# pasqal-io/Pulser

Hardware: NVIDIA H100
Metric: time-steps/s (1 ns sampling intervals of the Sequence evolved per second) (higher is better)
Workload: dtype f64 (complex128)

## Files before the change

### include/pulser_b200.h

```cpp
#ifndef PULSER_B200_H
#define PULSER_B200_H

#include <stdint.h>

#ifdef __cplusplus
extern "C" {
#endif

#define PB200_OK 0
#define PB200_ERR_INVALID -1
#define PB200_ERR_CUDA -2
#define PB200_ERR_UNSUPPORTED -3
#define PB200_ERR_STATE -4

#define PB200_MAX_QUDITS 40
#define PB200_MAX_DRIVES 3

typedef struct pb200_plan pb200_plan;

typedef struct pb200_drive_desc {
    int32_t state_to;
    int32_t state_from;
    int32_t uniform;
    int32_t reserved;
// ... 122 lines not shown
int pb200_shards_energy(pb200_plan** plans, int32_t count, double t_us,
                        double* energy, double* h2);
int pb200_shards_expect(pb200_plan** plans, int32_t count,
                        const pb200_op_terms* op, double* out);

int pb200_host_interpolate(const double* x, const double* y, int32_t n,
                           int32_t order, const double* tq, int32_t nq,
                           double* out);
int pb200_host_moments(const double* x, const double* y, int32_t n,
                       int32_t order, double a, double b, double* out4);
int pb200_host_taylor_fit(const double* x, const double* y, int32_t n,
                          int32_t order, double a, double h, int32_t p,
                          double* coeffs, double* resid);
int pb200_host_taylor_separable(const double* coef, const double* det,
                                int32_t n_traj, int32_t n_qudits,
                                int32_t n_times, int32_t* separable,
                                double* a_out, double* c_out, double* m_out);
int pb200_host_taylor_shapes(const double* coef, const double* det,
                             int32_t n_traj, int32_t n_qudits, int32_t n_times,
                             int32_t max_shapes, int32_t* n_shapes,
                             double* a_out, double* c_out, double* m_out);
int pb200_host_taylor_order(double h, const double* m, int32_t p, double tol,
                            int32_t* order_out, double* tail_out);
int pb200_host_chebyshev(double rho, double tol, double* out, int32_t cap,
                         int32_t* count);

#ifdef __cplusplus
}
#endif
#endif
```

### pulser_b200/_lib.py

```python
from __future__ import annotations

import ctypes as C
import os

_HERE = os.path.dirname(os.path.abspath(__file__))
LIB_PATH = os.path.join(_HERE, "libpulser_b200.so")

PB200_MAX_DRIVES = 3


class DriveDesc(C.Structure):
    _fields_ = [
        ("state_to", C.c_int32),
        ("state_from", C.c_int32),
        ("uniform", C.c_int32),
        ("reserved", C.c_int32),
    ]


class PlanDesc(C.Structure):
    _fields_ = [
        ("n_qudits", C.c_int32),
        ("dim", C.c_int32),
        ("n_times", C.c_int32),
# ... 100 lines not shown
        "pb200_bench_apply": (
            C.c_int, [vp, C.c_double, C.c_int32, dp, C.POINTER(C.c_int64)]),
        "pb200_plan_create_shard": (C.c_int, [C.POINTER(vp), C.POINTER(PlanDesc), C.c_int32, C.c_int32]),
        "pb200_shards_link": (C.c_int, [C.POINTER(vp), C.c_int32]),
        "pb200_shards_propagate": (
            C.c_int, [C.POINTER(vp), C.c_int32, C.c_double, C.c_double, C.POINTER(RunOpts), C.POINTER(RunStats)]),
        "pb200_shards_apply_h": (C.c_int, [C.POINTER(vp), C.c_int32, C.c_double, dp, dp]),
        "pb200_shards_energy": (C.c_int, [C.POINTER(vp), C.c_int32, C.c_double, dp, dp]),
        "pb200_shards_expect": (C.c_int, [C.POINTER(vp), C.c_int32, C.POINTER(OpTermsDesc), dp]),
        "pb200_host_interpolate": (
            C.c_int, [dp, dp, C.c_int32, C.c_int32, dp, C.c_int32, dp]),
        "pb200_host_moments": (
            C.c_int, [dp, dp, C.c_int32, C.c_int32, C.c_double, C.c_double, dp]),
        "pb200_host_chebyshev": (
            C.c_int, [C.c_double, C.c_double, dp, C.c_int32, C.POINTER(C.c_int32)]),
        "pb200_host_taylor_fit": (
            C.c_int, [dp, dp, C.c_int32, C.c_int32, C.c_double, C.c_double, C.c_int32, dp, dp]),
        "pb200_host_taylor_separable": (
            C.c_int, [dp, dp, C.c_int32, C.c_int32, C.c_int32, C.POINTER(C.c_int32), dp, dp, dp]),
        "pb200_host_taylor_shapes": (
            C.c_int, [dp, dp, C.c_int32, C.c_int32, C.c_int32, C.c_int32, C.POINTER(C.c_int32), dp, dp, dp]),
        "pb200_host_taylor_order": (
            C.c_int, [C.c_double, dp, C.c_int32, C.c_double, C.POINTER(C.c_int32), dp]),
    }
    for name, (res, args) in sig.items():
        fn = getattr(lib, name)
        fn.restype = res
        fn.argtypes = args
    return lib


EXPORTED_SYMBOLS = [
    "pb200_version", "pb200_last_error", "pb200_device_count",
    "pb200_plan_create", "pb200_plan_destroy", "pb200_plan_set_stream",
    "pb200_plan_set_interaction", "pb200_plan_set_xy", "pb200_plan_set_slm_mask", "pb200_plan_set_drive", "pb200_plan_set_dissipator", "pb200_plan_set_collapse",
    "pb200_plan_jump_counts", "pb200_state_set",
    "pb200_state_get", "pb200_state_probabilities", "pb200_state_norm2",
    "pb200_state_occupation", "pb200_state_correlation", "pb200_state_energy", "pb200_state_overlap", "pb200_state_expect", "pb200_state_sample", "pb200_state_copy", "pb200_state_device_ptr", "pb200_propagate", "pb200_apply_h",
    "pb200_coefficients_at", "pb200_bench_apply", "pb200_host_interpolate",
    "pb200_host_moments", "pb200_host_chebyshev", "pb200_host_taylor_fit", "pb200_host_taylor_order", "pb200_host_taylor_separable",
    "pb200_host_taylor_shapes",
    "pb200_plan_create_shard", "pb200_shards_link", "pb200_shards_propagate", "pb200_shards_apply_h", "pb200_shards_energy",
    "pb200_shards_expect",
]

lib = _load()


class PB200Error(RuntimeError):
    def __init__(self, code: int, msg: str):
        super().__init__(f"pulser_b200 error {code}: {msg}")
        self.code = code


def check(code: int) -> None:
    if code != 0:
        raise PB200Error(code, lib.pb200_last_error().decode("utf-8", "replace"))
```

### pulser_b200/csrc/kernels.cuh

```cuda
#pragma once
#include <cuda_runtime.h>
#include <stdint.h>
#include <type_traits>

namespace pb200 {

struct c2 { double x, y; };

__host__ __device__ inline c2 cmul(c2 a, c2 b) { return {a.x * b.x - a.y * b.y, a.x * b.y + a.y * b.x}; }
__host__ __device__ inline c2 cadd(c2 a, c2 b) { return {a.x + b.x, a.y + b.y}; }

struct PassGeom {
    int n_bits;
    int lo_bits;
    int hi_shift;
    int hi_bits;
    uint32_t tile_flip_mask;
    unsigned long long extra_mask;
    int first_pass;
};

struct StageCoef {
    c2 c_psi, c_b2, c_g;
};
// ... 1418 lines not shown
    for (long long idx = blockIdx.x * (long long)blockDim.x + threadIdx.x; idx < D;
         idx += (long long)gridDim.x * blockDim.x) {
        int cnt = 0;
        long long rem = off + idx;
        for (int k = 0; k < n; ++k) { cnt += ((int)(rem % dim) == rstate); rem /= dim; }
        const double v = dint[idx];
        unsigned long long* pmin = reinterpret_cast<unsigned long long*>(mins + cnt);
        unsigned long long old = *pmin;
        while (__longlong_as_double((long long)old) > v) {
            unsigned long long assumed = old;
            old = atomicCAS(pmin, assumed, (unsigned long long)__double_as_longlong(v));
            if (old == assumed) break;
        }
        unsigned long long* pmax = reinterpret_cast<unsigned long long*>(maxs + cnt);
        old = *pmax;
        while (__longlong_as_double((long long)old) < v) {
            unsigned long long assumed = old;
            old = atomicCAS(pmax, assumed, (unsigned long long)__double_as_longlong(v));
            if (old == assumed) break;
        }
    }
}

__global__ void bitstring_weights_kernel(const c2* psi, double* weights, long long D, int n, int dim, int one_digit,
                                         long long off) {
    for (long long s = blockIdx.x * (long long)blockDim.x + threadIdx.x; s < D;
         s += (long long)gridDim.x * blockDim.x) {
        const c2 v = psi[s];
        const double p = v.x * v.x + v.y * v.y;
        long long rem = off + s, b = 0;
        for (int k = n - 1; k >= 0; --k) {
            if ((int)(rem % dim) == one_digit) b |= 1LL << (n - 1 - k);
            rem /= dim;
        }
        if (dim == 2) weights[b & (D - 1)] = p;
        else atomicAdd(weights + b, p);
    }
}

__global__ void occupation_kernel(const c2* psi, double* occ, long long D, int n, int dim, int digit, long long off) {
    extern __shared__ double socc[];
    for (int i = threadIdx.x; i < n; i += blockDim.x) socc[i] = 0.0;
    __syncthreads();
    const long long traj = blockIdx.y;
    for (long long s = blockIdx.x * (long long)blockDim.x + threadIdx.x; s < D;
         s += (long long)gridDim.x * blockDim.x) {
// ... 451 lines not shown
```

### pulser_b200/csrc/plan.cu

```cuda
#include <cuda_runtime.h>

#include <algorithm>
#include <deque>
#include <map>
#include <memory>
#include <mutex>
#include <unordered_map>
#include <cmath>
#include <complex>
#include <cstdarg>
#include <cstdio>
#include <cstdlib>
#include <cstring>
#include <stdexcept>
#include <string>
#include <vector>

#include "../../include/pulser_b200.h"
#include "kernels.cuh"
#include "spline.hpp"
#include <cub/device/device_scan.cuh>
#include <nvtx3/nvToolsExt.h>
#include <random>

namespace pb200 {

// ... 230 lines not shown
    std::vector<double> times;
    int n = 0, dim = 0, B = 1;
    long long D = 0;
    int n_drives = 0;
    cudaStream_t stream = nullptr;
    struct OwnedStream {
        cudaStream_t s = nullptr;
        OwnedStream() = default;
        OwnedStream(const OwnedStream&) = delete;
        OwnedStream& operator=(const OwnedStream&) = delete;
        ~OwnedStream() { reset(); }
        void reset() {
            if (s) { cudaStreamSynchronize(s); cudaStreamDestroy(s); s = nullptr; }
        }
    } owned_stream;
    DevBuf<c2> buf[3];
    DevBuf<c2> aux[6];
    int cur = 0;
    DevBuf<double> dint;
    bool dint_shared = true;
    bool has_interaction = false;
    DevBuf<double> d_table;
    DevBuf<double> d_scratch;
    std::vector<std::vector<DriveTables>> tabs;
    std::vector<std::vector<bool>> tabs_set;
    std::vector<double> dmin_cnt, dmax_cnt;
    std::vector<double> dmin_traj, dmax_traj;
    bool state_set = false;
    int sm_count = 132;
    std::vector<std::vector<cplx>> diss_gen;
    DevBuf<c2> kry; int kry_cap = 0;
    DevBuf<double> d_kry;
    int m_last = 8;
    bool use_krylov = false;
    long long kry_iters = 0;
    bool has_diss = false;
    struct DissTaylor {
        bool ok = false;
        const char* why = "";
        c2 dw[4] = {}, df[4] = {};
        bool flip = false;
        double norm = 0.0;
    } diss_tay;
    std::vector<std::vector<cplx>> jump_ops;
    std::vector<std::vector<double>> jump_ldl;
    std::vector<std::vector<cplx>> jump_ldl_full;
// ... 1825 lines not shown
    return out;
}

static int taylor_order(double h, const std::vector<double>& mj, double tol, double& tail_out) {
    const int p = (int)mj.size() - 1;
    std::vector<double> y(1, 1.0);
    const int kcap = 1200;
    for (int k = 0; k < kcap; ++k) {
        double s = 0.0;
        for (int j = 0; j <= std::min(p, k); ++j) s += mj[j] * y[k - j];
        y.push_back(h * s / (k + 1));
        if (k > 8 && y.back() < 1e-40 && y.back() < y[k]) break;
    }
    double tail = 0.0;
    int kk = (int)y.size() - 1;
    for (; kk >= 1; --kk) {
        if (tail + y[kk] > tol) break;
        tail += y[kk];
    }
    tail_out = tail;
    return std::max(kk, 1);
}

static void launch_taylor_order(const Plan& P, bool tiled, const TaylorArgs& a, bool cplx) {
    const bool diss = a.n_pair > 0;
    if (!tiled) {
        const dim3 grid((unsigned)((P.D + 255) / 256), (unsigned)P.B);
        if (diss && !cplx) stage_d2_taylor_small_kernel<false, true><<<grid, 256, 0, P.stream>>>(a);
        else if (diss) fail(PB200_ERR_UNSUPPORTED, "no Taylor stage kernel for a dissipator with a complex drive");
        else if (cplx) stage_d2_taylor_small_kernel<true><<<grid, 256, 0, P.stream>>>(a);
        else stage_d2_taylor_small_kernel<false><<<grid, 256, 0, P.stream>>>(a);
        return;
    }
    const bool uniform = !a.table || (a.tab_shapes && P.tay.drive_uniform);
    const bool real_g = uniform && !cplx && a.unit.y == 0.0;
    const bool shard = a.shard_bits > 0;
    const int ns = a.tab_shapes ? PB200_TAYLOR_SMAX : uniform ? 0 : 1;
    for (const TaylorVariant& v : taylor_variants()) {
        if (v.uniform != uniform || v.real_g != real_g || v.shard != shard || v.ns != ns || v.cplx != cplx ||
            v.diss != diss)
            continue;
        const size_t tile = (size_t)16 << kTaylorTileBits;
        const size_t smem = v.smem == TaylorSmem::Shapes      ? taylor_shapes_smem(P.n)
                            : v.smem == TaylorSmem::TileTable ? tile + (size_t)d2_table_stride(P.n) * 8
                                                              : tile;
        launch_k(v.kernel, dim3((unsigned)(P.D >> kTaylorTileBits), uniform ? 1u : (unsigned)P.B),
// ... 11 lines not shown
    geo = passes[0];
    geo.n_bits = P.n;
    tiled = passes.size() == 1 && geo.first_pass && geo.hi_bits == 0 && geo.lo_bits == kTaylorTileBits;
    return tiled || P.n <= 16;
}

struct TaylorStep {
    double t = 0.0, h = 0.0;
    std::vector<double> om, th;
    std::vector<double> m[PB200_TAYLOR_SMAX];
    int p_om = 0, p_th = 0, p = 0;
    std::vector<double> gam;
    int K = 0;
    double phi = 0.0;
    int n_chi = 0, n_g = 0;
    int drive = 0;
    c2 unit{1.0, 0.0};
    std::vector<double> omi;
    int ring() const { return (n_chi - 1) + n_g * (drive == 2 ? 2 : 1) + 1; }
};

struct TaylorScheduler {
    Plan& P;
    double t_stop, eps = 1e-12, gtol, rate, rho_target, fit_total, fit_spent = 0.0, round2 = 0.0;
    double t, steps_len = 0.0, t_retry_len = 0.0, A_sum, C_sum[PB200_TAYLOR_SMAX], kRoundUnit = 0.05 * 1.1102230246251565e-16;
    int order, N, nt, ns;
    bool log_steps;
    pb200_run_stats st{};
    struct Fit { TaylorPoly om, omi, th, m[PB200_TAYLOR_SMAX]; double om_allow = 0.0; bool ok; };

    TaylorScheduler(Plan& P_, double t_start, double t_stop_, const pb200_run_opts* o) : P(P_), t_stop(t_stop_), t(t_start) {
        const double tlo = P.times.front(), thi = P.times.back();
        gtol = taylor_default_tol(P, o);
        rate = gtol / std::max(thi - tlo, 1e-30);
        constexpr double kTaylorRhoMax = 14.0;
        order = P.desc.interp_order;
        N = P.n;
        nt = (int)P.times.size();
        Plan::TaylorCache& C = P.tay;
        taylor_knot_widths(P);
        rho_target = kTaylorRhoMax;
        {
            double w_total = 0.0;
            for (int i = 0; i + 1 < nt; ++i) w_total += 0.5 * (C.w_knot[i] + C.w_knot[i + 1]) * (P.times[i + 1] - P.times[i]);
            for (int it = 0; it < 3; ++it) {
                const double n_est = std::max(w_total / std::max(rho_target, 1.0), 1.0);
                rho_target = std::min(kTaylorRhoMax, std::max(4.0, std::log(0.2 * gtol / (kRoundUnit * std::sqrt(n_est)))));
            }
        }
        A_sum = std::max(C.a_sum_max, 1e-300);
        ns = C.ns;
        for (int s = 0; s < PB200_TAYLOR_SMAX; ++s) C_sum[s] = std::max(C.c_sum_max[s], 1e-300);
        fit_total = 0.5 * rate * (t_stop - t_start);
        log_steps = env_int("PB200_TAYLOR_LOG", 0) != 0;
    }

    Fit fit_step(double a, double h, bool single_piece) {
        const Plan::TaylorCache& C = P.tay;
        Fit F; F.ok = false;
        const double budget = std::max(0.5 * rate * h, 0.02 * std::max(fit_total - fit_spent, 0.0));
        const double third = budget / (3.0 * h);
        auto one = [&](const PiecewiseCubic<double>& pc, TaylorPoly& out, double allow) {
            if (!single_piece) {
                out = taylor_fit(pc, P.times, order, a, h, PB200_TAYLOR_PMAX);
                if (out.resid > allow) return false;
            }
            for (int p = 0; p < PB200_TAYLOR_PMAX; ++p) {
                TaylorPoly f = taylor_fit(pc, P.times, order, a, h, p);
                if (f.resid <= allow || (single_piece && p >= 3)) { out = f; return true; }
            }
            if (single_piece) out = taylor_fit(pc, P.times, order, a, h, PB200_TAYLOR_PMAX);
            return true;
        };
        F.om_allow = third / A_sum;
        if (C.phase_moves) F.ok = one(C.om, F.om, 0.5 * F.om_allow) && one(C.om_im, F.omi, 0.5 * F.om_allow);
        else F.ok = one(C.om, F.om, F.om_allow);
        F.ok = F.ok && one(P.tabs[0][0].det[0], F.th, third / N);
        for (int s = 0; s < ns && F.ok; ++s) F.ok = one(C.shape[s], F.m[s], third / ns / C_sum[s]);
        for (int s = ns; s < PB200_TAYLOR_SMAX; ++s) { F.m[s].c.assign(1, 0.0); F.m[s].resid = 0.0; }
        return F;
    }

    double candidate_end(int i0) {
        const Plan::TaylorCache& C = P.tay;
        double b = t, acc = 0.0, cur = t;
        int i = i0;
        while (i < nt - 1) {
            const double e1 = std::min(P.times[i + 1], t_stop);
            const double w = std::max(C.w_knot[i], C.w_knot[i + 1]);
            const double need = w * (e1 - cur);
            if (acc + need > rho_target) {
                if (i == i0 || acc == 0.0) b = cur + (rho_target - acc) / std::max(w, 1e-300);
                else b = cur;
                break;
            }
            acc += need; cur = e1; b = e1; ++i;
            if (e1 >= t_stop - eps) break;
        }
        b = std::min(b, t_stop);
        if (t_retry_len > 0.0) { b = std::min(b, t + t_retry_len); t_retry_len = 0.0; }
        if (b <= t + eps) b = std::min(P.times[i0 + 1], t_stop);
        return b;
    }

    Fit longest_fit(int i0, double& b) {
        const bool single = b <= P.times[i0 + 1] + eps;
        Fit F = fit_step(t, b - t, single);
        if (F.ok || single) return F;
        int lo_keep = 0, hi_keep = find_piece(P.times, b - eps) - i0;
        Fit Flo; bool have_lo = false;
        while (hi_keep - lo_keep > 1) {
            const int mid = (lo_keep + hi_keep) / 2;
            const double bm = P.times[i0 + 1 + mid];
            Fit Fm = fit_step(t, bm - t, false);
            if (Fm.ok) { lo_keep = mid; Flo = Fm; have_lo = true; } else hi_keep = mid;
        }
        b = P.times[i0 + 1 + lo_keep];
        return have_lo ? Flo : fit_step(t, b - t, lo_keep == 0);
    }

    double classify_drive(Fit& F, int& drive, c2& unit) const {
        auto coef = [](const std::vector<double>& c, size_t j) { return j < c.size() ? c[j] : 0.0; };
        auto poly = [](const std::vector<double>& c, double u) {
// ... 50 lines not shown

    void centres_and_bounds(const Fit& F, bool cplx, int p_om, int p, std::vector<double>& gam, std::vector<double>& mj) const {
        auto th_c = [&](int j) { return j < (int)F.th.c.size() ? F.th.c[j] : 0.0; };
        auto m_c = [&](int q, int j) { return j < (int)F.m[q].c.size() ? F.m[q].c[j] : 0.0; };
        auto om_abs = [&](int j) {
            const double x = j < (int)F.om.c.size() ? F.om.c[j] : 0.0;
            if (!cplx) return std::fabs(x);
            return std::hypot(x, j < (int)F.omi.c.size() ? F.omi.c[j] : 0.0);
        };
        gam.assign(p + 1, 0.0); mj.assign(p + 1, 0.0);
        double c0, hw0, mv[PB200_TAYLOR_SMAX];
        for (int q = 0; q < PB200_TAYLOR_SMAX; ++q) mv[q] = m_c(q, 0);
        taylor_bounds(P, cplx ? om_abs(0) : F.om.c[0], F.th.c[0], mv, c0, hw0);
        gam[0] = c0; mj[0] = hw0 + P.diss_tay.norm;
        for (int j = 1; j <= p; ++j) {
            const double thj = th_c(j), omj = j <= p_om ? om_abs(j) : 0.0;
            gam[j] = -thj * 0.5 * N;
            double mm = 0.0;
            for (int q = 0; q < ns; ++q) mm += std::fabs(m_c(q, j)) * C_sum[q];
            mj[j] = std::fabs(thj) * 0.5 * N + mm + std::fabs(omj) * A_sum;
        }
    }

    void record(TaylorStep& s, const Fit& F, const std::vector<double>& mj, int p_m, double om_resid, double rho) {
        double trunc_bound = 0.0;
        s.K = taylor_order(s.h, mj, std::max(1e-15, 0.1 * rate * s.h), trunc_bound);
        st.n_applies += s.K; st.n_exponentials += 1; ++st.n_steps;
        if (log_steps)
            fprintf(stderr, "taylor step t=%.6f h_ns=%.3f p_om=%d p_th=%d p_m=%d K=%d ring=%d rho=%.3f resid=%.2e/%.2e/%.2e drive=%s\n",
                    s.t, s.h * 1e3, s.p_om, s.p_th, p_m, s.K, s.ring() + 1, mj[0] * s.h, om_resid, F.th.resid, F.m[0].resid,
                    s.drive == 2 ? "cplx" : s.drive == 1 ? "rot" : "real");
        st.max_rho = std::max(st.max_rho, rho);
        double fit_m = 0.0;
        for (int q = 0; q < ns; ++q) fit_m += C_sum[q] * F.m[q].resid;
        const double fit_err = s.h * (A_sum * om_resid + N * F.th.resid + fit_m);
        st.err_estimate += trunc_bound + fit_err;
        fit_spent += fit_err;
        { const double r = kRoundUnit * std::exp(std::min(rho, 40.0)); round2 += r * r; }
        steps_len += s.h;
    }

    bool next(TaylorStep& s) {
        while (t < t_stop - eps) {
            const int i0 = find_piece(P.times, t + eps);
            double b = candidate_end(i0);
            Fit F = longest_fit(i0, b);
            const double h = b - t;
            int drive = 0;
            c2 unit = P.tay.unit;
            const double om_resid = P.tay.phase_moves ? classify_drive(F, drive, unit) : F.om.resid;
            const int p_m = trim(F, drive == 2);
            const int p_om = std::max((int)F.om.c.size(), drive == 2 ? (int)F.omi.c.size() : 0) - 1;
            const int p_th = std::max((int)F.th.c.size() - 1, p_m);
            const int p = std::max(p_om, p_th);
            std::vector<double> gam, mj;
            centres_and_bounds(F, drive == 2, p_om, p, gam, mj);
            double rho = 0.0;
            for (int j = 0; j <= p; ++j) rho += mj[j] / (j + 1);
            rho *= h;
            if (rho > 1.12 * rho_target && h > 1e-9) {
                t_retry_len = h * rho_target / rho;
                continue;
            }
            s.t = t; s.h = h;
            s.om = F.om.c; s.th = F.th.c;
            for (int q = 0; q < PB200_TAYLOR_SMAX; ++q) s.m[q] = F.m[q].c;
            s.p_om = p_om; s.p_th = p_th; s.p = p;
            s.gam = gam;
            s.n_chi = p_th + 2;
            s.n_g = p_om >= 1 ? p_om + 1 : 0;
            s.drive = drive; s.unit = unit;
            s.omi = drive == 2 ? F.omi.c : std::vector<double>();
            double phi = 0.0;
            for (int j = 0; j <= p; ++j) phi += gam[j] / (j + 1);
            s.phi = phi * h;
            record(s, F, mj, p_m, om_resid, rho);
            t = b;
            return true;
        }
        return false;
    }

    pb200_run_stats finish(double gpu_ms, long long launches) const {
        pb200_run_stats out = st;
        out.gpu_ms = gpu_ms;
        out.n_launches = launches;
        const double hi_mean = (P.times.back() - P.times.front()) / std::max(nt - 1, 1);
        out.mean_step_samples = out.n_steps ? steps_len / out.n_steps / hi_mean : 0.0;
        out.err_estimate += std::sqrt(round2);
        out.integrator = 3;
        return out;
    }
};

struct TaylorRing {
    std::vector<c2*> chi, gr, gr2;
    DevBuf<c2>* acc_slot = nullptr;
};

static void taylor_grow_ring(Plan& P, int need) {
// ... 117 lines not shown
                    a.peer[q] = R[peer].chi[k % s.n_chi];
                    if (!first) CUDA_CHECK(cudaStreamWaitEvent(P.stream, order_ev.ev[peer], 0));
                }
                launch_taylor_order(P, tiled, a, s.drive == 2);
                ++launches;
            }
            for (int r = 0; r < count && sb; ++r) CUDA_CHECK(cudaEventRecord(order_ev.ev[r], use(r).stream));
            first = false;
        }
        CUDA_CHECK(cudaGetLastError());
        for (int r = 0; r < count; ++r) std::swap(G[r]->buf[G[r]->cur], *R[r].acc_slot);
    }
    float ms_max = 0.f;
    for (int r = 0; r < count; ++r) CUDA_CHECK(cudaEventRecord(t1.ev[r], use(r).stream));
    for (int r = 0; r < count; ++r) {
        CUDA_CHECK(cudaEventSynchronize(t1.ev[r]));
        float ms = 0.f;
        CUDA_CHECK(cudaEventElapsedTime(&ms, t0.ev[r], t1.ev[r]));
        ms_max = std::max(ms_max, ms);
    }
    return ms_max;
}

static void propagate_taylor(Plan& P, double t_start, double t_stop, const pb200_run_opts* o, pb200_run_stats* stats) {
    PassGeom geo;
    bool tiled = false;
    if (!taylor_geometry(P, geo, tiled)) fail(PB200_ERR_UNSUPPORTED, "Taylor propagator: unsupported register size");
    ensure_aux_buffers(P);
    TaylorScheduler S(P, t_start, t_stop, o);
    long long launches = 0;
    const float ms = taylor_launch_steps({&P}, geo, tiled, [&S](TaylorStep& s) { return S.next(s); }, launches);
    if (stats) *stats = S.finish(ms, launches);
}

static ExpParams params_at(const Plan& P, double t) {
    ExpParams E;
    const int N = P.n, B = P.B, nd = P.n_drives;
    E.g.assign((size_t)B * nd * N, cplx(0)); E.th.assign((size_t)B * nd * N, 0.0); E.w = 1.0;
    if (P.has_slm) E.wc = eval_at(P.slm_coef, P.times, t, P.desc.interp_order);
    for (int tr = 0; tr < B; ++tr)
        for (int q = 0; q < nd; ++q) {
            const DriveTables& T = P.tabs[tr][q];
            const int rows = (int)T.coef.size();
            for (int k = 0; k < N; ++k) {
                const int r = rows == 1 ? 0 : k;
                E.g[pidx(P, tr, q, k)] = eval_at(T.coef[r], P.times, t, P.desc.interp_order);
                E.th[pidx(P, tr, q, k)] = eval_at(T.det[r], P.times, t, P.desc.interp_order);
            }
        }
    return E;
}

static void apply_h_device(Plan& P, double t, const c2* in, c2* out, long long& launches) {
    const bool d2path = is_d2path(P);
    const bool uniform = d2path && P.all_uniform() && P.B == 1;
// ... 958 lines not shown
            mn = std::min(mn, G[i]->dmin_traj[0]); mx = std::max(mx, G[i]->dmax_traj[0]);
        }
        for (Plan* P : G) { P->dmin_cnt = mins; P->dmax_cnt = maxs; P->dmin_traj[0] = mn; P->dmax_traj[0] = mx; }
    }
    for (Plan* P : G) { P->tay.w_knot.clear(); P->group = G; }
    PB200_CATCH
}

int pb200_shards_propagate(pb200_plan** plans, int32_t count, double t_start, double t_stop, const pb200_run_opts* o,
                           pb200_run_stats* stats) {
    PB200_TRY
    NvtxRange nvtx_range("pb200_shards_propagate");
    const std::vector<Plan*> G = shard_group(plans, count, "pb200_shards_propagate");
    if (o && ((o->integrator != 0 && o->integrator != 3) || o->max_step_samples > 0 || o->tol < 0.0))
        fail(PB200_ERR_UNSUPPORTED, "pb200_shards_propagate: shards run the Taylor propagator only (integrator 0 or 3, "
                                    "max_step_samples = 0, tol >= 0)");
    for (int r = 0; r < count; ++r)
        if (!G[r]->state_set) fail(PB200_ERR_STATE, "pb200_shards_propagate: no state set on shard %d", r);
    Plan& P0 = *G[0];
    const double tlo = P0.times.front(), thi = P0.times.back(), eps = 1e-12;
    if (t_start < tlo - eps || t_stop > thi + eps || t_stop < t_start)
        fail(PB200_ERR_INVALID, "pb200_shards_propagate: [%g, %g] outside sampling times [%g, %g]", t_start, t_stop, tlo, thi);
    t_start = std::max(t_start, tlo); t_stop = std::min(t_stop, thi);
    PassGeom geo;
    bool tiled = false;
    taylor_geometry(P0, geo, tiled);
    TaylorScheduler S(P0, t_start, t_stop, o);
    std::vector<TaylorStep> steps;
    for (TaylorStep s; S.next(s);) steps.push_back(s);
    int need = 0;
    for (const TaylorStep& s : steps) need = std::max(need, s.ring());
    for (Plan* P : G) {
        CUDA_CHECK(cudaSetDevice(P->desc.device));
        try {
            taylor_grow_ring(*P, need);
        } catch (const Error& e) {
            fail(PB200_ERR_CUDA, "pb200_shards_propagate: this call needs the state and %d more state-sized buffers per shard, "
                                 "%lld bytes each (%d amplitudes x 16 B) besides the 8 B/amplitude interaction diagonal: %s",
                 need, (long long)(16 * P->D), (int)P->D, e.what());
        }
    }
    long long launches = 0;
    size_t i = 0;
    auto next = [&](TaylorStep& s) {
        if (i == steps.size()) return false;
        s = steps[i++];
        return true;
    };
    const float ms = taylor_launch_steps(G, geo, tiled, next, launches);
    if (stats) *stats = S.finish(ms, launches);
    PB200_CATCH
}

int pb200_shards_apply_h(pb200_plan** plans, int32_t count, double t_us, const double* in, double* out) {
    PB200_TRY
    NvtxRange nvtx_range("pb200_shards_apply_h");
    if (!in || !out) fail(PB200_ERR_INVALID, "null argument");
    const std::vector<Plan*> G = shard_group(plans, count, "pb200_shards_apply_h");
    std::vector<c2*> bin(count), bout(count);
    for (int r = 0; r < count; ++r) {
        Plan& P = *G[r];
        bin[r] = P.buf[(P.cur + 1) % 3].get(); bout[r] = P.buf[(P.cur + 2) % 3].get();
        CUDA_CHECK(cudaSetDevice(P.desc.device));
        CUDA_CHECK(cudaMemcpyAsync(bin[r], in + (size_t)2 * P.D * r, sizeof(c2) * (size_t)P.D, cudaMemcpyHostToDevice, P.stream));
    }
    shards_apply_h(G, t_us, bin, bout);
    for (int r = 0; r < count; ++r) {
        Plan& P = *G[r];
        CUDA_CHECK(cudaSetDevice(P.desc.device));
        CUDA_CHECK(cudaMemcpyAsync(out + (size_t)2 * P.D * r, bout[r], sizeof(c2) * (size_t)P.D, cudaMemcpyDeviceToHost, P.stream));
    }
    shards_sync(G);
    PB200_CATCH
// ... 155 lines not shown
    *n_shapes = F.ok ? F.ns : -1;
    if (F.ok) {
        if (a_out)
            for (size_t x = 0; x < F.a.size(); ++x) { a_out[2 * x] = F.a[x].real(); a_out[2 * x + 1] = F.a[x].imag(); }
        if (c_out)
            for (size_t x = 0; x < (size_t)n_traj * N; ++x)
                for (size_t s = 0; s < S; ++s) c_out[x * S + s] = (int)s < F.ns ? F.c[x * F.ns + s] : 0.0;
        if (m_out)
            for (size_t s = 0; s < S; ++s)
                for (size_t i = 0; i < nt; ++i) m_out[s * nt + i] = (int)s < F.ns ? F.m[s][i] : 0.0;
    }
    PB200_CATCH
}

int pb200_host_taylor_order(double h, const double* m, int32_t p, double tol, int32_t* order_out, double* tail_out) {
    PB200_TRY
    if (!m || !order_out || p < 0 || p > PB200_TAYLOR_PMAX) fail(PB200_ERR_INVALID, "bad argument");
    double tail = 0.0;
    *order_out = taylor_order(h, std::vector<double>(m, m + p + 1), tol, tail);
    if (tail_out) *tail_out = tail;
    PB200_CATCH
}

int pb200_host_chebyshev(double rho, double tol, double* out, int32_t cap, int32_t* count) {
    PB200_TRY
    if (!out || !count) fail(PB200_ERR_INVALID, "bad argument");
    std::vector<cplx> a = chebyshev_exp_coeffs(rho, tol);
    *count = (int32_t)a.size();
    for (int i = 0; i < (int)a.size() && i < cap; ++i) { out[2 * i] = a[i].real(); out[2 * i + 1] = a[i].imag(); }
    PB200_CATCH
}

}
```

Baseline: 20370.

## Choose Taylor step size and order from per-excitation-sector norm majorants

Adds a sector-resolved majorant bound for the Taylor propagator. When the drive is uniform and the interaction is shared, each step's order and length come from the state's norms per Rydberg-excitation count. These norms are computed on the GPU by a new binning kernel and copied back asynchronously through pinned slots and events. The aim is longer steps and fewer Hamiltonian applies than the scalar bound allows. In exchange, the host scheduler now waits on device norms, which can stall the launch pipeline. Sharded propagation also changes from pre-planning all steps to scheduling them on the fly.

```diff
diff --git a/experiments/sector_majorant_study.py b/experiments/sector_majorant_study.py
--- /dev/null
+++ b/experiments/sector_majorant_study.py
@@ -0,0 +1,159 @@
+from __future__ import annotations
+
+import sys
+import time
+
+import numpy as np
+from scipy.integrate import solve_ivp
+
+sys.path.insert(0, ".")
+sys.path.insert(0, "experiments")
+from taylor_time_study import build, kinks, poly_fit, xtot
+
+RHO = 14.0
+TOL = 1e-8
+
+
+def tail_order(y, tol):
+    tail, k = 0.0, len(y) - 1
+    while k >= 1 and tail + y[k] <= tol:
+        tail += y[k]
+        k -= 1
+    return max(k, 1)
+
+
+def scalar_majorant(h, m, kmax=400):
+    y = [1.0]
+    for k in range(kmax):
+        y.append(h * sum(m[j] * y[k - j] for j in range(min(len(m) - 1, k) + 1)) / (k + 1))
+    return np.array(y)
+
+
+def sector_majorant(h, d, om, y0, kmax=400):
+    n = len(y0) - 1
+    x = np.sqrt((np.arange(n + 1) + 1.0) * (n - np.arange(n + 1)))[:-1]
+    Y = [np.asarray(y0, float)]
+    for k in range(kmax):
+        s = np.zeros(n + 1)
+        for j in range(min(len(om) - 1, k) + 1):
+            v = Y[k - j]
+            s += d[j] * v
+            s[1:] += om[j] * x * v[:-1]
+            s[:-1] += om[j] * x * v[1:]
+        Y.append(h * s / (k + 1))
+        if k > 20 and Y[-1].sum() < 1e-40:
+            break
+    return np.array([np.linalg.norm(v) for v in Y])
+
+
+def run(n, rule):
+    spec, t, om, de, dint, cnt = build(n)
+    D = 1 << n
+    exc = cnt.astype(int)
+    psi = np.zeros(D, complex)
+    psi[D - 1] = 1.0
+    T = t[-1]
+    rate = TOL / T
+    kk = set(kinks(t, [om, de]))
+    dmin = np.array([dint[exc == c].min() for c in range(n + 1)])
+    dmax = np.array([dint[exc == c].max() for c in range(n + 1)])
+    a, applies, steps = 0.0, 0, 0
+    while a < T - 1e-12:
+        i0 = int(np.searchsorted(t, a + 1e-12, side="right") - 1)
+        i1 = i0 + 1
+        while i1 < len(t) - 1 and i1 not in kk:
+            i1 += 1
+        end_fit = t[i1]
+
+        def coeffs(h):
+            co, r1 = poly_fit(om, a, h, 3)
+            cd, r2 = poly_fit(de, a, h, 3)
+            return co, cd
+
+        def fits(h):
+            if a + h <= t[i0 + 1] + 1e-12:
+                return True
+            return (poly_fit(om, a, h, 3)[1] + poly_fit(de, a, h, 3)[1]) * n <= 0.5 * rate * h
+
+        def sector_ranges(cd):
+            return dmin - cd[0] * np.arange(n + 1), dmax - cd[0] * np.arange(n + 1)
+
+        def scalar(h):
+            co, cd = coeffs(h)
+            lo, hi = sector_ranges(cd)
+            W = 0.5 * (hi.max() - lo.min()) + abs(co[0]) * n
+            m = [W] + [abs(cd[j]) * n / 2 + abs(co[j]) * n for j in (1, 2, 3)]
+            y = scalar_majorant(h, m)
+            return tail_order(y, 0.1 * rate * h), 0.5 * (hi.max() + lo.min()), co, cd, h * sum(mj / (j + 1) for j, mj in enumerate(m))
+
+        h = min(end_fit - a, T - a)
+        while not fits(h):
+            h = max(0.5 * h, min(t[i0 + 1] - a, T - a))
+        h_fit = h
+        while True:
+            K, c0, co, cd, rho = scalar(h)
+            if rho <= RHO * 1.0001:
+                break
+            h *= RHO / rho
+        if rule == "sector":
+            y0 = np.array([np.linalg.norm(psi[exc == c]) for c in range(n + 1)])
+            best = None
+            for f in (1.0, 1.3, 1.6, 2.0, 2.5, 3.0, 4.0):
+                hc = min(f * h, h_fit)
+                if not fits(hc):
+                    break
+                co, cd = coeffs(hc)
+                lo, hi = sector_ranges(cd)
+                for g in np.linspace(lo.min(), hi.max(), 25):
+                    d0 = np.maximum(hi - g, g - lo)
+                    dj = [np.abs(cd[j]) * np.abs(np.arange(n + 1) - n / 2) for j in (1, 2, 3)]
+                    y = sector_majorant(hc, [d0] + dj, np.abs(co), y0)
+                    if y.max() > np.exp(RHO):
+                        continue
+                    Kc = tail_order(y, 0.1 * rate * hc)
+                    if best is None or Kc / hc < best[0]:
+                        best = (Kc / hc, hc, Kc, g, co, cd)
+                if hc >= h_fit:
+                    break
+            if best is not None:
+                _, h, K, c0, co, cd = best
+        gj = [c0] + [-cd[j] * n / 2 for j in (1, 2, 3)]
+        chis, Gs = [psi], []
+        acc = psi.copy()
+        for k in range(K):
+            Gs.append(xtot(chis[k], n))
+            new = (dint - cd[0] * cnt - c0) * chis[k] + co[0] * Gs[k]
+            for j in range(1, min(3, k) + 1):
+                new += (-cd[j] * cnt - gj[j]) * chis[k - j] + co[j] * Gs[k - j]
+            new *= -1j * h / (k + 1)
+            chis.append(new)
+            if len(chis) > 5:
+                chis[k - 4] = Gs[k - 4] = None
+            acc += new
+        psi = acc * np.exp(-1j * h * sum(g / (j + 1) for j, g in enumerate(gj)))
+        applies += K
+        steps += 1
+        a += h
+    return psi, applies / (T * 1e3), steps, (spec, t, om, de, dint, cnt)
+
+
+def main():
+    ns = [int(x) for x in sys.argv[1:]] or [12, 14, 16, 18]
+    for n in ns:
+        t0 = time.time()
+        ps, aps, ss, (spec, t, om, de, dint, cnt) = run(n, "scalar")
+        pv, apv, sv, _ = run(n, "sector")
+        line = (f"N={n}: scalar {aps:.3f} applies/ns ({ss} steps), sector {apv:.3f} ({sv} steps): "
+                f"{aps / apv:.2f}x fewer; |psi_scalar - psi_sector| {np.linalg.norm(ps - pv):.1e}")
+        if n <= 14:
+            D = 1 << n
+            psi0 = np.zeros(D, complex)
+            psi0[D - 1] = 1.0
+            rhs = lambda tt, y: -1j * ((dint - de(tt) * cnt) * y + om(tt) * xtot(y, n))
+            ref = solve_ivp(rhs, (0.0, t[-1]), psi0, method="DOP853", rtol=1e-12, atol=1e-14, max_step=2e-3).y[:, -1]
+            line += f"; error vs DOP853: scalar {np.linalg.norm(ps - ref):.1e}, sector {np.linalg.norm(pv - ref):.1e}"
+        print(line + f"  [{time.time() - t0:.0f} s]", flush=True)
+
+
+if __name__ == "__main__":
+    main()
diff --git a/include/pulser_b200.h b/include/pulser_b200.h
--- a/include/pulser_b200.h
+++ b/include/pulser_b200.h
@@ -168,6 +168,11 @@
                              double* a_out, double* c_out, double* m_out);
 int pb200_host_taylor_order(double h, const double* m, int32_t p, double tol,
                             int32_t* order_out, double* tail_out);
+int pb200_host_taylor_sector_order(double h, int32_t n, int32_t p,
+                                   const double* d, const double* om,
+                                   const double* y0, double tol, double gmax,
+                                   int32_t* order_out, double* tail_out,
+                                   double* g_out);
 int pb200_host_chebyshev(double rho, double tol, double* out, int32_t cap,
                          int32_t* count);
 
diff --git a/pulser_b200/_lib.py b/pulser_b200/_lib.py
--- a/pulser_b200/_lib.py
+++ b/pulser_b200/_lib.py
@@ -146,6 +146,9 @@
             C.c_int, [dp, dp, C.c_int32, C.c_int32, C.c_int32, C.c_int32, C.POINTER(C.c_int32), dp, dp, dp]),
         "pb200_host_taylor_order": (
             C.c_int, [C.c_double, dp, C.c_int32, C.c_double, C.POINTER(C.c_int32), dp]),
+        "pb200_host_taylor_sector_order": (
+            C.c_int, [C.c_double, C.c_int32, C.c_int32, dp, dp, dp, C.c_double, C.c_double, C.POINTER(C.c_int32), dp,
+                      dp]),
     }
     for name, (res, args) in sig.items():
         fn = getattr(lib, name)
@@ -163,7 +166,7 @@
     "pb200_state_occupation", "pb200_state_correlation", "pb200_state_energy", "pb200_state_overlap", "pb200_state_expect", "pb200_state_sample", "pb200_state_copy", "pb200_state_device_ptr", "pb200_propagate", "pb200_apply_h",
     "pb200_coefficients_at", "pb200_bench_apply", "pb200_host_interpolate",
     "pb200_host_moments", "pb200_host_chebyshev", "pb200_host_taylor_fit", "pb200_host_taylor_order", "pb200_host_taylor_separable",
-    "pb200_host_taylor_shapes",
+    "pb200_host_taylor_shapes", "pb200_host_taylor_sector_order",
     "pb200_plan_create_shard", "pb200_shards_link", "pb200_shards_propagate", "pb200_shards_apply_h", "pb200_shards_energy",
     "pb200_shards_expect",
 ]
diff --git a/pulser_b200/csrc/kernels.cuh b/pulser_b200/csrc/kernels.cuh
--- a/pulser_b200/csrc/kernels.cuh
+++ b/pulser_b200/csrc/kernels.cuh
@@ -1464,6 +1464,21 @@
     }
 }
 
+__global__ void sector_norm2_kernel(const c2* __restrict__ psi, long long D, int n, int from_is_one, int ones_hi,
+                                    double* out) {
+    __shared__ double bins[65];
+    for (int c = threadIdx.x; c <= n; c += blockDim.x) bins[c] = 0.0;
+    __syncthreads();
+    for (long long idx = blockIdx.x * (long long)blockDim.x + threadIdx.x; idx < D;
+         idx += (long long)gridDim.x * blockDim.x) {
+        const int ones = __popcll((unsigned long long)idx) + ones_hi;
+        const c2 v = psi[idx];
+        atomicAdd(&bins[from_is_one ? ones : n - ones], v.x * v.x + v.y * v.y);
+    }
+    __syncthreads();
+    for (int c = threadIdx.x; c <= n; c += blockDim.x) atomicAdd(out + c, bins[c]);
+}
+
 __global__ void bitstring_weights_kernel(const c2* psi, double* weights, long long D, int n, int dim, int one_digit,
                                          long long off) {
     for (long long s = blockIdx.x * (long long)blockDim.x + threadIdx.x; s < D;
diff --git a/pulser_b200/csrc/plan.cu b/pulser_b200/csrc/plan.cu
--- a/pulser_b200/csrc/plan.cu
+++ b/pulser_b200/csrc/plan.cu
@@ -2,6 +2,7 @@
 
 #include <algorithm>
 #include <deque>
+#include <functional>
 #include <map>
 #include <memory>
 #include <mutex>
@@ -278,6 +279,19 @@
     bool has_interaction = false;
     DevBuf<double> d_table;
     DevBuf<double> d_scratch;
+    struct SectorSlots {
+        static constexpr int kSlots = 4;
+        double* host = nullptr;
+        cudaEvent_t ev[kSlots] = {};
+        SectorSlots() = default;
+        SectorSlots(const SectorSlots&) = delete;
+        SectorSlots& operator=(const SectorSlots&) = delete;
+        ~SectorSlots() {
+            for (cudaEvent_t e : ev) if (e) cudaEventDestroy(e);
+            if (host) cudaFreeHost(host);
+        }
+    };
+    std::unique_ptr<SectorSlots> sec;
     std::vector<std::vector<DriveTables>> tabs;
     std::vector<std::vector<bool>> tabs_set;
     std::vector<double> dmin_cnt, dmax_cnt;
@@ -2149,6 +2163,51 @@
     return std::max(kk, 1);
 }
 
+static bool sector_order(double h, int N, int p, const double* d, const double* om, const double* y0, double tol,
+                         double gmax, int& K, double& tail_out, double& G, int K_fixed = 0, double* csum = nullptr) {
+    const int S = N + 1, kcap = 1200;
+    std::vector<double> x(S, 0.0), Y(y0, y0 + S), y(1, 0.0);
+    for (int c = 0; c < N; ++c) x[c] = std::sqrt((c + 1.0) * (N - c));
+    for (int c = 0; c < S; ++c) y[0] += y0[c] * y0[c];
+    y[0] = std::sqrt(y[0]);
+    G = y[0];
+    bool rest = false;
+    for (int k = 0; k < kcap && !rest; ++k) {
+        Y.resize(Y.size() + S, 0.0);
+        double* out = Y.data() + (size_t)(k + 1) * S;
+        for (int j = 0; j <= std::min(p, k); ++j) {
+            const double* v = Y.data() + (size_t)(k - j) * S;
+            const double* dj = d + (size_t)j * S;
+            for (int c = 0; c < S; ++c) {
+                double s = dj[c] * v[c];
+                if (c > 0) s += om[j] * x[c - 1] * v[c - 1];
+                if (c < N) s += om[j] * x[c] * v[c + 1];
+                out[c] += s;
+            }
+        }
+        double n2 = 0.0;
+        for (int c = 0; c < S; ++c) { out[c] *= h / (k + 1); n2 += out[c] * out[c]; }
+        y.push_back(std::sqrt(n2));
+        G = std::max(G, y.back());
+        if (G > gmax) return false;
+        rest = k > 8 && y.back() < 1e-3 * tol && y.back() < 0.5 * y[k];
+    }
+    double tail = rest ? y.back() : 0.0;
+    int kk = (int)y.size() - 1;
+    for (; kk >= 1; --kk) {
+        if (K_fixed > 0 ? kk <= K_fixed : tail + y[kk] > tol) break;
+        tail += y[kk];
+    }
+    tail_out = tail;
+    K = K_fixed > 0 ? K_fixed : std::max(kk, 1);
+    if (csum)
+        for (int c = 0; c < S; ++c) {
+            csum[c] = 0.0;
+            for (int k = 0; k <= K && (size_t)k * S < Y.size(); ++k) csum[c] += Y[(size_t)k * S + c];
+        }
+    return true;
+}
+
 static void launch_taylor_order(const Plan& P, bool tiled, const TaylorArgs& a, bool cplx) {
     const bool diss = a.n_pair > 0;
     if (!tiled) {
@@ -2206,6 +2265,9 @@
 
 struct TaylorScheduler {
     Plan& P;
+    bool sector = false;
+    std::function<void(int, std::vector<double>&)> norms;
+    int n_done = 0;
     double t_stop, eps = 1e-12, gtol, rate, rho_target, fit_total, fit_spent = 0.0, round2 = 0.0;
     double t, steps_len = 0.0, t_retry_len = 0.0, A_sum, C_sum[PB200_TAYLOR_SMAX], kRoundUnit = 0.05 * 1.1102230246251565e-16;
     int order, N, nt, ns;
@@ -2237,6 +2299,8 @@
         for (int s = 0; s < PB200_TAYLOR_SMAX; ++s) C_sum[s] = std::max(C.c_sum_max[s], 1e-300);
         fit_total = 0.5 * rate * (t_stop - t_start);
         log_steps = env_int("PB200_TAYLOR_LOG", 0) != 0;
+        sector = C.drive_uniform && P.has_interaction && P.dint_shared &&
+                 P.desc.drives[0].state_from == P.desc.rydberg_state && (int)P.dmin_cnt.size() == N + 1;
     }
 
     Fit fit_step(double a, double h, bool single_piece) {
@@ -2265,7 +2329,7 @@
         return F;
     }
 
-    double candidate_end(int i0) {
+    double candidate_end(int i0, double rho_t) const {
         const Plan::TaylorCache& C = P.tay;
         double b = t, acc = 0.0, cur = t;
         int i = i0;
@@ -2273,8 +2337,8 @@
             const double e1 = std::min(P.times[i + 1], t_stop);
             const double w = std::max(C.w_knot[i], C.w_knot[i + 1]);
             const double need = w * (e1 - cur);
-            if (acc + need > rho_target) {
-                if (i == i0 || acc == 0.0) b = cur + (rho_target - acc) / std::max(w, 1e-300);
+            if (acc + need > rho_t) {
+                if (i == i0 || acc == 0.0) b = cur + (rho_t - acc) / std::max(w, 1e-300);
                 else b = cur;
                 break;
             }
@@ -2282,7 +2346,7 @@
             if (e1 >= t_stop - eps) break;
         }
         b = std::min(b, t_stop);
-        if (t_retry_len > 0.0) { b = std::min(b, t + t_retry_len); t_retry_len = 0.0; }
+        if (t_retry_len > 0.0) b = std::min(b, t + t_retry_len);
         if (b <= t + eps) b = std::min(P.times[i0 + 1], t_stop);
         return b;
     }
@@ -2379,9 +2443,8 @@
         }
     }
 
-    void record(TaylorStep& s, const Fit& F, const std::vector<double>& mj, int p_m, double om_resid, double rho) {
-        double trunc_bound = 0.0;
-        s.K = taylor_order(s.h, mj, std::max(1e-15, 0.1 * rate * s.h), trunc_bound);
+    void record(TaylorStep& s, const Fit& F, const std::vector<double>& mj, int p_m, double om_resid, double rho,
+                double trunc_bound, double r_round) {
         st.n_applies += s.K; st.n_exponentials += 1; ++st.n_steps;
         if (log_steps)
             fprintf(stderr, "taylor step t=%.6f h_ns=%.3f p_om=%d p_th=%d p_m=%d K=%d ring=%d rho=%.3f resid=%.2e/%.2e/%.2e drive=%s\n",
@@ -2393,46 +2456,195 @@
         const double fit_err = s.h * (A_sum * om_resid + N * F.th.resid + fit_m);
         st.err_estimate += trunc_bound + fit_err;
         fit_spent += fit_err;
-        { const double r = kRoundUnit * std::exp(std::min(rho, 40.0)); round2 += r * r; }
+        round2 += r_round * r_round;
         steps_len += s.h;
+    }
+
+    struct Cand {
+        double b, h, om_resid, rho;
+        Fit F;
+        int drive = 0, p_m, p_om, p_th, p;
+        c2 unit;
+        std::vector<double> gam, mj;
+    };
+    Cand candidate(int i0, double b) {
+        Cand c;
+        c.F = longest_fit(i0, b);
+        c.b = b; c.h = b - t;
+        c.unit = P.tay.unit;
+        c.om_resid = P.tay.phase_moves ? classify_drive(c.F, c.drive, c.unit) : c.F.om.resid;
+        c.p_m = trim(c.F, c.drive == 2);
+        c.p_om = std::max((int)c.F.om.c.size(), c.drive == 2 ? (int)c.F.omi.c.size() : 0) - 1;
+        c.p_th = std::max((int)c.F.th.c.size() - 1, c.p_m);
+        c.p = std::max(c.p_om, c.p_th);
+        centres_and_bounds(c.F, c.drive == 2, c.p_om, c.p, c.gam, c.mj);
+        c.rho = 0.0;
+        for (int j = 0; j <= c.p; ++j) c.rho += c.mj[j] / (j + 1);
+        c.rho *= c.h;
+        return c;
+    }
+
+    void commit(TaylorStep& s, const Cand& c, int K, double trunc_bound, double r_round) {
+        s.t = t; s.h = c.h;
+        s.om = c.F.om.c; s.th = c.F.th.c;
+        for (int q = 0; q < PB200_TAYLOR_SMAX; ++q) s.m[q] = c.F.m[q].c;
+        s.p_om = c.p_om; s.p_th = c.p_th; s.p = c.p;
+        s.gam = c.gam;
+        s.n_chi = c.p_th + 2;
+        s.n_g = c.p_om >= 1 ? c.p_om + 1 : 0;
+        s.drive = c.drive; s.unit = c.unit;
+        s.omi = c.drive == 2 ? c.F.omi.c : std::vector<double>();
+        double phi = 0.0;
+        for (int j = 0; j <= c.p; ++j) phi += c.gam[j] / (j + 1);
+        s.phi = phi * c.h;
+        s.K = K;
+        record(s, c.F, c.mj, c.p_m, c.om_resid, c.rho, trunc_bound, r_round);
+        t = c.b;
+        ++n_done;
+    }
+
+    void sector_rows(const Cand& c, std::vector<double>& lo, std::vector<double>& hi, std::vector<double>& dj,
+                     std::vector<double>& om) const {
+        const Plan::TaylorCache& C = P.tay;
+        const Fit& F = c.F;
+        auto m_c = [&](int q, int j) { return j < (int)F.m[q].c.size() ? F.m[q].c[j] : 0.0; };
+        lo.assign(N + 1, 0.0); hi.assign(N + 1, 0.0);
+        std::vector<double> small(N + 1, 0.0), large(N + 1, 0.0);
+        if (ns) {
+            std::vector<double> e(N, 0.0);
+            for (int k = 0; k < N; ++k)
+                for (int q = 0; q < ns; ++q) e[k] += C.c[(size_t)k * C.ns + q] * m_c(q, 0);
+            std::sort(e.begin(), e.end());
+            for (int k = 1; k <= N; ++k) { small[k] = small[k - 1] + e[k - 1]; large[k] = large[k - 1] + e[N - k]; }
+        }
+        for (int k = 0; k <= N; ++k) {
+            lo[k] = P.dmin_cnt[k] - F.th.c[0] * k - large[k];
+            hi[k] = P.dmax_cnt[k] - F.th.c[0] * k - small[k];
+        }
+        dj.assign((size_t)(c.p + 1) * (N + 1), 0.0);
+        om.assign(c.p + 1, 0.0);
+        for (int j = 0; j <= c.p; ++j) {
+            const double x = j < (int)F.om.c.size() ? F.om.c[j] : 0.0;
+            const double y = c.drive == 2 && j < (int)F.omi.c.size() ? F.omi.c[j] : 0.0;
+            om[j] = j <= c.p_om ? std::hypot(x, y) : 0.0;
+            if (j == 0) continue;
+            const double thj = j < (int)F.th.c.size() ? F.th.c[j] : 0.0;
+            double mm = 0.0;
+            for (int q = 0; q < ns; ++q) mm += std::fabs(m_c(q, j)) * C_sum[q];
+            for (int k = 0; k <= N; ++k) dj[(size_t)j * (N + 1) + k] = std::fabs(thj) * std::fabs(k - 0.5 * N) + mm;
+        }
+    }
+
+    bool sector_eval(const Cand& c, double g0, double gmax, std::vector<double>& dj, const std::vector<double>& lo,
+                     const std::vector<double>& hi, const std::vector<double>& om, const std::vector<double>& y0,
+                     int& K, double& tail, double& G, int K_fixed = 0, double* csum = nullptr) const {
+        for (int k = 0; k <= N; ++k)
+            dj[k] = P.dmin_cnt[k] > P.dmax_cnt[k] ? 0.0 : std::max(hi[k] - g0, g0 - lo[k]);
+        return sector_order(c.h, N, c.p, dj.data(), om.data(), y0.data(), std::max(1e-15, 0.1 * rate * c.h), gmax, K,
+                            tail, G, K_fixed, csum);
+    }
+
+    std::vector<double> sector_start(int i) const {
+        std::vector<double> y;
+        norms(i, y);
+        for (double& v : y) {
+            int e = 0;
+            const double m = std::frexp(std::sqrt(std::max(v, 0.0)) * (1.0 + 1e-12), &e);
+            v = std::ldexp(std::ceil(m * 4096.0) / 4096.0, e);
+        }
+        return y;
+    }
+
+    Cand pend;
+    double pend_g0 = 0.0;
+    int pend_K = 0, pend_i = -1;
+    std::vector<double> after_pend(const std::vector<double>& y0) const {
+        std::vector<double> lo, hi, dj, om, out(N + 1);
+        sector_rows(pend, lo, hi, dj, om);
+        int K; double tail, G;
+        sector_eval(pend, pend_g0, 1e300, dj, lo, hi, om, y0, K, tail, G, pend_K, out.data());
+        for (double& v : out) v = std::min(v, 1.0 + 1e-9);
+        return out;
+    }
+
+    int sector_next(int i0, TaylorStep& s) {
+        const std::vector<double> yp = sector_start(std::max(n_done - 1, 0));
+        double top = 0.0;
+        for (int c = (3 * N + 3) / 4; c <= N; ++c) top += yp[c] * yp[c];
+        if (top > 1e-6) { pend_i = -1; return 2; }
+        std::vector<Cand> cands;
+        for (double f : {1.0, 1.4, 2.0, 2.8, 4.0}) {
+            const double b = candidate_end(i0, f * rho_target);
+            if (!cands.empty() && b <= cands.back().b + eps) break;
+            Cand c = candidate(i0, b);
+            if (!cands.empty() && c.b <= cands.back().b + eps) break;
+            cands.push_back(std::move(c));
+        }
+        t_retry_len = 0.0;
+        const std::vector<double> y0 = pend_i >= 0 && pend_i == n_done - 1 ? after_pend(yp) : sector_start(n_done);
+        const double gmax = std::exp(rho_target);
+        std::vector<double> lo, hi, dj, om;
+        auto search = [&](const Cand& c) {
+            sector_rows(c, lo, hi, dj, om);
+            double a = 1e300, b = -1e300;
+            for (int k = 0; k <= N; ++k)
+                if (P.dmin_cnt[k] <= P.dmax_cnt[k]) { a = std::min(a, lo[k]); b = std::max(b, hi[k]); }
+            auto Gat = [&](double g) {
+                int K; double tail, G;
+                return sector_eval(c, g, 1e300, dj, lo, hi, om, y0, K, tail, G) ? G : 1e300;
+            };
+            const double r = 0.5 * (std::sqrt(5.0) - 1.0);
+            double x1 = b - r * (b - a), x2 = a + r * (b - a), f1 = Gat(x1), f2 = Gat(x2);
+            for (int it = 0; it < 16; ++it) {
+                if (f1 < f2) { b = x2; x2 = x1; f2 = f1; x1 = b - r * (b - a); f1 = Gat(x1); }
+                else { a = x1; x1 = x2; f1 = f2; x2 = a + r * (b - a); f2 = Gat(x2); }
+            }
+            const double g = f1 < f2 ? x1 : x2;
+            return Gat(c.gam[0]) <= std::min(f1, f2) ? c.gam[0] : g;
+        };
+        std::vector<double> centres = {search(cands.front())};
+        if (cands.size() > 1) centres.push_back(search(cands.back()));
+        int best = -1, bestK = 0;
+        double best_rate = 1e300, best_g0 = 0.0, best_tail = 0.0, best_G = 0.0;
+        for (size_t i = 0; i < cands.size(); ++i) {
+            sector_rows(cands[i], lo, hi, dj, om);
+            for (double g0 : centres) {
+                int K; double tail, G;
+                if (!sector_eval(cands[i], g0, gmax, dj, lo, hi, om, y0, K, tail, G)) continue;
+                if (K / cands[i].h < best_rate) {
+                    best = (int)i; best_rate = K / cands[i].h; bestK = K; best_g0 = g0; best_tail = tail; best_G = G;
+                }
+            }
+        }
+        if (best < 0) {
+            t_retry_len = 0.5 * cands[0].h;
+            return 0;
+        }
+        Cand& c = cands[best];
+        c.gam[0] = best_g0;
+        pend = c; pend_g0 = best_g0; pend_K = bestK; pend_i = n_done;
+        commit(s, c, bestK, best_tail, kRoundUnit * best_G);
+        return 1;
     }
 
     bool next(TaylorStep& s) {
         while (t < t_stop - eps) {
             const int i0 = find_piece(P.times, t + eps);
-            double b = candidate_end(i0);
-            Fit F = longest_fit(i0, b);
-            const double h = b - t;
-            int drive = 0;
-            c2 unit = P.tay.unit;
-            const double om_resid = P.tay.phase_moves ? classify_drive(F, drive, unit) : F.om.resid;
-            const int p_m = trim(F, drive == 2);
-            const int p_om = std::max((int)F.om.c.size(), drive == 2 ? (int)F.omi.c.size() : 0) - 1;
-            const int p_th = std::max((int)F.th.c.size() - 1, p_m);
-            const int p = std::max(p_om, p_th);
-            std::vector<double> gam, mj;
-            centres_and_bounds(F, drive == 2, p_om, p, gam, mj);
-            double rho = 0.0;
-            for (int j = 0; j <= p; ++j) rho += mj[j] / (j + 1);
-            rho *= h;
-            if (rho > 1.12 * rho_target && h > 1e-9) {
-                t_retry_len = h * rho_target / rho;
+            if (sector) {
+                const int r = sector_next(i0, s);
+                if (r == 1) return true;
+                if (r == 0) continue;
+            }
+            const double b = candidate_end(i0, rho_target);
+            t_retry_len = 0.0;
+            const Cand c = candidate(i0, b);
+            if (c.rho > 1.12 * rho_target && c.h > 1e-9) {
+                t_retry_len = c.h * rho_target / c.rho;
                 continue;
             }
-            s.t = t; s.h = h;
-            s.om = F.om.c; s.th = F.th.c;
-            for (int q = 0; q < PB200_TAYLOR_SMAX; ++q) s.m[q] = F.m[q].c;
-            s.p_om = p_om; s.p_th = p_th; s.p = p;
-            s.gam = gam;
-            s.n_chi = p_th + 2;
-            s.n_g = p_om >= 1 ? p_om + 1 : 0;
-            s.drive = drive; s.unit = unit;
-            s.omi = drive == 2 ? F.omi.c : std::vector<double>();
-            double phi = 0.0;
-            for (int j = 0; j <= p; ++j) phi += gam[j] / (j + 1);
-            s.phi = phi * h;
-            record(s, F, mj, p_m, om_resid, rho);
-            t = b;
+            double trunc_bound = 0.0;
+            const int K = taylor_order(c.h, c.mj, std::max(1e-15, 0.1 * rate * c.h), trunc_bound);
+            commit(s, c, K, trunc_bound, kRoundUnit * std::exp(std::min(c.rho, 40.0)));
             return true;
         }
         return false;
@@ -2596,15 +2808,71 @@
     return ms_max;
 }
 
-static void propagate_taylor(Plan& P, double t_start, double t_stop, const pb200_run_opts* o, pb200_run_stats* stats) {
+struct SectorNorms {
+    static constexpr int kSlots = Plan::SectorSlots::kSlots, kBins = 65;
+    const std::vector<Plan*>& G;
+    const int n;
+    explicit SectorNorms(const std::vector<Plan*>& G_) : G(G_), n(G_[0]->n) {}
+    void init() {
+        for (Plan* P : G) {
+            if (P->sec) continue;
+            CUDA_CHECK(cudaSetDevice(P->desc.device));
+            std::unique_ptr<Plan::SectorSlots> S(new Plan::SectorSlots());
+            CUDA_CHECK(cudaMallocHost(&S->host, sizeof(double) * kSlots * kBins));
+            for (cudaEvent_t& e : S->ev) CUDA_CHECK(cudaEventCreateWithFlags(&e, cudaEventDisableTiming));
+            P->sec = std::move(S);
+        }
+    }
+    void enqueue(int i) {
+        const int k = i % kSlots;
+        for (size_t r = 0; r < G.size(); ++r) {
+            Plan& P = *G[r];
+            if (G.size() > 1) CUDA_CHECK(cudaSetDevice(P.desc.device));
+            double* d = P.d_scratch.get() + (size_t)k * (n + 1);
+            const long long blocks = std::min<long long>((P.D + 255) / 256, (long long)P.sm_count * 8);
+            CUDA_CHECK(cudaMemsetAsync(d, 0, sizeof(double) * (n + 1), P.stream));
+            sector_norm2_kernel<<<(unsigned)std::max<long long>(blocks, 1), 256, 0, P.stream>>>(
+                P.buf[P.cur].get(), P.D, n, P.desc.drives[0].state_from, __builtin_popcount((unsigned)P.shard), d);
+            CUDA_CHECK(cudaGetLastError());
+            CUDA_CHECK(cudaMemcpyAsync(P.sec->host + (size_t)k * kBins, d, sizeof(double) * (n + 1),
+                                       cudaMemcpyDeviceToHost, P.stream));
+            CUDA_CHECK(cudaEventRecord(P.sec->ev[k], P.stream));
+        }
+    }
+    void fetch(int i, std::vector<double>& out) const {
+        const int k = i % kSlots;
+        out.assign(n + 1, 0.0);
+        for (const Plan* P : G) {
+            CUDA_CHECK(cudaEventSynchronize(P->sec->ev[k]));
+            for (int c = 0; c <= n; ++c) out[c] += P->sec->host[(size_t)k * kBins + c];
+        }
+    }
+};
+
+static pb200_run_stats propagate_taylor_group(const std::vector<Plan*>& G, double t_start, double t_stop,
+                                              const pb200_run_opts* o) {
     PassGeom geo;
     bool tiled = false;
-    if (!taylor_geometry(P, geo, tiled)) fail(PB200_ERR_UNSUPPORTED, "Taylor propagator: unsupported register size");
+    if (!taylor_geometry(*G[0], geo, tiled)) fail(PB200_ERR_UNSUPPORTED, "Taylor propagator: unsupported register size");
+    TaylorScheduler S(*G[0], t_start, t_stop, o);
+    SectorNorms SN(G);
+    if (S.sector) {
+        SN.init();
+        S.norms = [&SN](int i, std::vector<double>& y) { SN.fetch(i, y); };
+    }
+    long long launches = 0;
+    auto next = [&](TaylorStep& s) {
+        if (S.sector) SN.enqueue(S.n_done);
+        return S.next(s);
+    };
+    const float ms = taylor_launch_steps(G, geo, tiled, next, launches);
+    return S.finish(ms, launches);
+}
+
+static void propagate_taylor(Plan& P, double t_start, double t_stop, const pb200_run_opts* o, pb200_run_stats* stats) {
     ensure_aux_buffers(P);
-    TaylorScheduler S(P, t_start, t_stop, o);
-    long long launches = 0;
-    const float ms = taylor_launch_steps({&P}, geo, tiled, [&S](TaylorStep& s) { return S.next(s); }, launches);
-    if (stats) *stats = S.finish(ms, launches);
+    const pb200_run_stats st = propagate_taylor_group({&P}, t_start, t_stop, o);
+    if (stats) *stats = st;
 }
 
 static ExpParams params_at(const Plan& P, double t) {
@@ -3609,33 +3877,8 @@
     if (t_start < tlo - eps || t_stop > thi + eps || t_stop < t_start)
         fail(PB200_ERR_INVALID, "pb200_shards_propagate: [%g, %g] outside sampling times [%g, %g]", t_start, t_stop, tlo, thi);
     t_start = std::max(t_start, tlo); t_stop = std::min(t_stop, thi);
-    PassGeom geo;
-    bool tiled = false;
-    taylor_geometry(P0, geo, tiled);
-    TaylorScheduler S(P0, t_start, t_stop, o);
-    std::vector<TaylorStep> steps;
-    for (TaylorStep s; S.next(s);) steps.push_back(s);
-    int need = 0;
-    for (const TaylorStep& s : steps) need = std::max(need, s.ring());
-    for (Plan* P : G) {
-        CUDA_CHECK(cudaSetDevice(P->desc.device));
-        try {
-            taylor_grow_ring(*P, need);
-        } catch (const Error& e) {
-            fail(PB200_ERR_CUDA, "pb200_shards_propagate: this call needs the state and %d more state-sized buffers per shard, "
-                                 "%lld bytes each (%d amplitudes x 16 B) besides the 8 B/amplitude interaction diagonal: %s",
-                 need, (long long)(16 * P->D), (int)P->D, e.what());
-        }
-    }
-    long long launches = 0;
-    size_t i = 0;
-    auto next = [&](TaylorStep& s) {
-        if (i == steps.size()) return false;
-        s = steps[i++];
-        return true;
-    };
-    const float ms = taylor_launch_steps(G, geo, tiled, next, launches);
-    if (stats) *stats = S.finish(ms, launches);
+    const pb200_run_stats st = propagate_taylor_group(G, t_start, t_stop, o);
+    if (stats) *stats = st;
     PB200_CATCH
 }
 
@@ -3837,6 +4080,20 @@
     PB200_CATCH
 }
 
+int pb200_host_taylor_sector_order(double h, int32_t n, int32_t p, const double* d, const double* om, const double* y0,
+                                   double tol, double gmax, int32_t* order_out, double* tail_out, double* g_out) {
+    PB200_TRY
+    if (!d || !om || !y0 || !order_out || n < 1 || n > 64 || p < 0 || p > PB200_TAYLOR_PMAX)
+        fail(PB200_ERR_INVALID, "bad argument");
+    int K = 0;
+    double tail = 0.0, G = 0.0;
+    const bool ok = sector_order(h, n, p, d, om, y0, tol, gmax, K, tail, G);
+    *order_out = ok ? K : 0;
+    if (tail_out) *tail_out = ok ? tail : 0.0;
+    if (g_out) *g_out = G;
+    PB200_CATCH
+}
+
 int pb200_host_chebyshev(double rho, double tol, double* out, int32_t cap, int32_t* count) {
     PB200_TRY
     if (!out || !count) fail(PB200_ERR_INVALID, "bad argument");
```

After: 22690, median of 6. 1.11x the previous value.
